# rtqichen/torchdiffeq

Measured on AMD Instinct MI355X. Metric: dopri5 RK-stages/sec at batch=65536x dim=128 (end-to-end adaptive trial steps incl. func, error norm, read-back and hos~, higher is better.
Workload: dtype f32; 1 GPU; BASELINE.json configs[1]: dopri5 adaptive, linear ODE dy/dt=Ay, batch=65536 x dim=128 fp32 per GPU, rtol=1e-7 atol=1e-9; global_batch=65536, rows_per_gpu=65536, dim=128, parallelism=batch-sharded x1, accepted=1937, rejected=2, lookahead=True, hip_graph=False

## Files before the change

include/tdeq_hip.h:

```cpp
#ifndef TDEQ_HIP_H
#define TDEQ_HIP_H

#include <stddef.h>
#include <stdint.h>

#ifdef __cplusplus
extern "C" {
#endif

#define TDEQ_ABI_VERSION 28
#define TDEQ_F32 0
#define TDEQ_F64 1
#define TDEQ_C64 2
#define TDEQ_C128 3
#define TDEQ_BF16 4
#define TDEQ_F16 5
#define TDEQ_MAX_TERMS 14
#define TDEQ_MAX_SUM_TERMS 8
#define TDEQ_MAX_DENSE_OUTPUTS 16
#define TDEQ_MAX_SEGMENTS 4096
#define TDEQ_INLINE_SEGMENTS 16
#define TDEQ_CHUNK_QUANTUM 1024

#define TDEQ_EINVAL (-1)
#define TDEQ_EWORKSPACE (-2)

typedef struct tdeq_segment {
    int64_t chunk_start;
    int64_t numel;
    double rtol;
    double atol;
} tdeq_segment;

#define TDEQ_MAX_STAGE_TIMES 16
typedef struct tdeq_step_ctrl {
    double t0;
    double dt;
    double safety;
    double ifactor;
    double dfactor;
// ... 63 lines not shown
int tdeq_stage_combine_multi_dev(const tdeq_multi_out* outs, int n_out, const void* y0, const void* acc_in,
                                 const void* const* k, int n_terms, const double* ctrl_dev, int64_t n, int dtype,
                                 void* stream);
int tdeq_stage_combine_multi_timed(const tdeq_multi_out* outs, int n_out, const void* y0, const void* acc_in,
                                   const void* const* k, int n_terms, double dt, int64_t n, int dtype, void* stream,
                                   void* start_event, void* stop_event);

int tdeq_error_norm_partial_ctrl(const void* err_partial, const void* y0, const void* y1, const void* const* k,
                                 const double* coef, int n_terms, double dt, const tdeq_segment* segs,
                                 const void* segs_dev, int n_seg, int64_t chunk, int64_t n_chunks, double* out_sumsq,
                                 double* out_nonfinite, const tdeq_step_ctrl* ctrl, double* out_ctrl, double* ctrl_dev,
                                 void* next_times, int state_in_dev, void* copy_last_k, void* workspace,
                                 size_t workspace_bytes, int dtype, void* stream);
int tdeq_stage_combine_sel(void* out, const void* y_acc, const void* f_acc, const void* y_rej, const void* f_rej,
                           double coef, const double* ctrl_dev, int64_t n, int dtype, void* stream);

int tdeq_step_controller(const double* sums, const double* nonfinite, const tdeq_segment* segs, const void* segs_dev,
                         int n_seg, double* out_sumsq, double* out_nonfinite, const tdeq_step_ctrl* ctrl,
                         double* out_ctrl, double* ctrl_dev, void* next_times, int state_in_dev, int dtype,
                         void* stream);

int tdeq_stage_combine_dev(void* out, void* err_out, const void* y0, const void* const* k, const double* coef,
                           const double* err_coef, int n_terms, const double* ctrl_dev, int64_t n, int dtype,
                           void* stream);
int tdeq_step_commit(void* y_prev, void* f_prev, void* y_cur, void* f_cur, const void* y1, const void* f1,
                     const double* ctrl_dev, int64_t n, int dtype, void* stream);

int tdeq_init_norms(int mode, const void* a, const void* b, const void* yscale,
                    const tdeq_segment* segs, const void* segs_dev, int n_seg, int64_t chunk,
                    int64_t n_chunks, double* out_sumsq, double* out_nonfinite, void* workspace, size_t workspace_bytes,
// ... 149 lines not shown
```

torchdiffeq_amd/_native.py:

```python
from __future__ import annotations

import contextlib
import ctypes
import functools
import math
import os
import threading
from typing import List, Optional, Sequence, Tuple

import numpy as np
import torch

TDEQ_ABI_VERSION = 28
TDEQ_F32, TDEQ_F64 = 0, 1
TDEQ_C64, TDEQ_C128 = 2, 3
TDEQ_BF16, TDEQ_F16 = 4, 5
TDEQ_MAX_TERMS = 14
TDEQ_INLINE_SEGMENTS = 16
TDEQ_CHUNK_QUANTUM = 1024
TDEQ_MAX_STAGE_TIMES = 16
TDEQ_MAX_DENSE_OUTPUTS = 16
TDEQ_MAX_MULTI_OUT = 4
TDEQ_MAX_GATHER = 4

_LIB_NAME = "libtdeq_hip.so"
_LIB_PATH = os.path.join(os.path.dirname(os.path.abspath(__file__)), _LIB_NAME)

_c_void_pp = ctypes.POINTER(ctypes.c_void_p)
# ... 83 lines not shown
                                                      ctypes.c_void_p, _c_void_pp, ctypes.c_int, ctypes.c_double,
                                                      ctypes.c_int64, ctypes.c_int, ctypes.c_void_p, ctypes.c_void_p,
                                                      ctypes.c_void_p]),
    "tdeq_error_norm_partial": (ctypes.c_int, [ctypes.c_void_p, ctypes.c_void_p, ctypes.c_void_p, _c_void_pp,
                                               _c_double_p, ctypes.c_int, ctypes.c_double, ctypes.POINTER(Segment),
                                               ctypes.c_void_p, ctypes.c_int, ctypes.c_int64, ctypes.c_int64,
                                               ctypes.c_void_p, ctypes.c_void_p, ctypes.c_void_p,
                                               ctypes.c_size_t, ctypes.c_int, ctypes.c_void_p]),
    "tdeq_error_norm_partial_ctrl": (ctypes.c_int, [ctypes.c_void_p, ctypes.c_void_p, ctypes.c_void_p, _c_void_pp,
                                                    _c_double_p, ctypes.c_int, ctypes.c_double,
                                                    ctypes.POINTER(Segment), ctypes.c_void_p, ctypes.c_int, ctypes.c_int64,
                                                    ctypes.c_int64, ctypes.c_void_p, ctypes.c_void_p,
                                                    ctypes.POINTER(StepCtrl), ctypes.c_void_p, ctypes.c_void_p,
                                                    ctypes.c_void_p, ctypes.c_int, ctypes.c_void_p, ctypes.c_void_p, ctypes.c_size_t,
                                                    ctypes.c_int, ctypes.c_void_p]),
    "tdeq_step_controller": (ctypes.c_int, [ctypes.c_void_p, ctypes.c_void_p, ctypes.POINTER(Segment), ctypes.c_void_p,
                                            ctypes.c_int, ctypes.c_void_p, ctypes.c_void_p,
                                            ctypes.POINTER(StepCtrl), ctypes.c_void_p, ctypes.c_void_p,
                                            ctypes.c_void_p, ctypes.c_int, ctypes.c_int, ctypes.c_void_p]),
    "tdeq_stage_combine_dev": (ctypes.c_int, [ctypes.c_void_p, ctypes.c_void_p, ctypes.c_void_p, _c_void_pp,
                                              _c_double_p, _c_double_p, ctypes.c_int, ctypes.c_void_p, ctypes.c_int64,
                                              ctypes.c_int, ctypes.c_void_p]),
    "tdeq_step_commit": (ctypes.c_int, [ctypes.c_void_p, ctypes.c_void_p, ctypes.c_void_p, ctypes.c_void_p,
                                        ctypes.c_void_p, ctypes.c_void_p, ctypes.c_void_p, ctypes.c_int64,
                                        ctypes.c_int, ctypes.c_void_p]),
    "tdeq_stage_combine_sel": (ctypes.c_int, [ctypes.c_void_p, ctypes.c_void_p, ctypes.c_void_p, ctypes.c_void_p,
                                              ctypes.c_void_p, ctypes.c_double, ctypes.c_void_p, ctypes.c_int64,
                                              ctypes.c_int, ctypes.c_void_p]),
    "tdeq_init_norms": (ctypes.c_int, [ctypes.c_int, ctypes.c_void_p, ctypes.c_void_p, ctypes.c_void_p,
                                       ctypes.POINTER(Segment), ctypes.c_void_p, ctypes.c_int,
# ... 178 lines not shown
        self.n_chunks = max(1, math.ceil(total / chunk))
        arr = (Segment * self.n_seg)()
        for i, (off, numel, rtol, atol) in enumerate(segments):
            assert off % chunk == 0, "segment offsets must be chunk aligned"
            arr[i] = Segment(off // chunk, numel, float(rtol), float(atol))
        self.segs = arr
        self.segs_dev = None
        if self.n_seg > TDEQ_INLINE_SEGMENTS:
            raw = np.frombuffer(bytes(arr), dtype=np.uint8).copy()
            self.segs_dev = torch.from_numpy(raw).to(device)
        self.workspace = torch.empty(3 * self.n_chunks, dtype=torch.float64, device=device)
        self.workspace_bytes = self.workspace.numel() * 8
        self.pinned = pinned
        self.expect = ()
        if pinned:
            self.out = torch.zeros(3 * self.n_seg + 4, dtype=torch.float64, device="cpu", pin_memory=True)
            self.out_np = self.out.numpy()
            self.out_bits = self.out_np.view(np.uint64)
        else:
            self.out = torch.zeros(3 * self.n_seg + 4, dtype=torch.float64, device=device)
            self.out_np = None
        self.out_ptr = self.out.data_ptr()
        self.bad_ptr = self.out_ptr + 16 * self.n_seg
        self.ctrl_ptr = self.out_ptr + 24 * self.n_seg
        self.ctrl_dev = torch.zeros(4, dtype=torch.float64, device=device)


class HipKernels:

    name = "hip"

    _SENTINEL = np.uint64(0x7FF8DEADBEEF0001)
    _POLL_TIMEOUT_S = 5.0

    def __init__(self, lib: ctypes.CDLL):
        self.lib = lib
        mode = os.environ.get("TDEQ_READBACK", "poll")
        if mode not in ("poll", "pinned", "copy"):
            raise ValueError(f"TDEQ_READBACK={mode!r}: expected poll | pinned | copy")
        self._mode = mode
        self._pinned = mode in ("poll", "pinned")

    def _arm(self, plan: "NormPlan", n_sum: int, ctrl: bool = False) -> None:
        if self._mode == "poll" and plan.pinned:
            n = plan.n_seg
            plan.out_bits[:n_sum * n] = self._SENTINEL
            plan.out_bits[2 * n:3 * n + (4 if ctrl else 0)] = self._SENTINEL
            plan.expect = ((0, n_sum * n), (2 * n, 3 * n + (4 if ctrl else 0)))

    _raw_stream = staticmethod(getattr(torch._C, "_cuda_getCurrentRawStream", None))
    _cur_device = staticmethod(getattr(torch._C, "_cuda_getDevice", None))

    @classmethod
    def _stream(cls) -> int:
        if cls._raw_stream is not None and cls._cur_device is not None:
            return cls._raw_stream(cls._cur_device())
        return torch.cuda.current_stream().cuda_stream

    _TLS = threading.local()
    _COEF_ARRAYS: dict = {}
    _PACK_TABLES: dict = {}

    @classmethod
# ... 212 lines not shown

    def error_norm_partial_ctrl(self, plan: NormPlan, err_partial, y0, y1, ks, coefs, dt: float, ctrl: StepCtrl,
                                next_times, state_in_dev: bool = False, copy_last_to=None) -> None:
        n = len(ks)
        ptrs = (ctypes.c_void_p * max(n, 1))(*[k.data_ptr() for k in ks])
        cf = (ctypes.c_double * max(n, 1))(*coefs)
        self._arm(plan, 1, ctrl=True)
        _check(self.lib.tdeq_error_norm_partial_ctrl(
            err_partial.data_ptr(), y0.data_ptr(), y1.data_ptr(), ptrs, cf, n, dt, plan.segs,
            plan.segs_dev.data_ptr() if plan.segs_dev is not None else None, plan.n_seg, plan.chunk,
            plan.n_chunks, plan.out_ptr, plan.bad_ptr, ctypes.byref(ctrl), plan.ctrl_ptr, plan.ctrl_dev.data_ptr(),
            next_times.data_ptr(), 1 if state_in_dev else 0, None if copy_last_to is None else copy_last_to.data_ptr(),
            plan.workspace.data_ptr(), plan.workspace_bytes, dtype_code(y0.dtype), self._stream()),
            "tdeq_error_norm_partial_ctrl")

    def step_controller(self, plan: NormPlan, sums_plan: NormPlan, numel_plan: NormPlan, ctrl: StepCtrl, next_times,
                        dtype: torch.dtype, state_in_dev: bool = False) -> None:
        assert not sums_plan.pinned and sums_plan.n_seg == plan.n_seg == numel_plan.n_seg
        self._arm(plan, 1, ctrl=True)
        _check(self.lib.tdeq_step_controller(
            sums_plan.out_ptr, sums_plan.bad_ptr, numel_plan.segs,
            numel_plan.segs_dev.data_ptr() if numel_plan.segs_dev is not None else None, plan.n_seg, plan.out_ptr,
            plan.bad_ptr, ctypes.byref(ctrl), plan.ctrl_ptr, plan.ctrl_dev.data_ptr(), next_times.data_ptr(),
            1 if state_in_dev else 0, dtype_code(dtype), self._stream()), "tdeq_step_controller")

    def read_ctrl(self, plan: NormPlan) -> Tuple[bool, float, float, List[float]]:
        n = plan.n_seg
        v = self._read_out(plan)
        return v[3 * n] != 0.0, v[3 * n + 1], v[3 * n + 2], v[2 * n:3 * n]

    def stage_combine_dev(self, out, err_out, y0, ks, coefs, err_coefs, plan: NormPlan) -> None:
        ptrs, cf, n = self._terms(ks, coefs)
        ef = None if err_coefs is None else (ctypes.c_double * n)(*err_coefs)
        _check(self.lib.tdeq_stage_combine_dev(out.data_ptr(), None if err_out is None else err_out.data_ptr(),
                                               y0.data_ptr(), ptrs, cf, ef, n, plan.ctrl_dev.data_ptr(), y0.numel(),
                                               dtype_code(y0.dtype), self._stream()), "tdeq_stage_combine_dev")

    def step_commit(self, y_prev, f_prev, y_cur, f_cur, y1, f1, plan: NormPlan) -> None:
        _check(self.lib.tdeq_step_commit(y_prev.data_ptr(), f_prev.data_ptr(), y_cur.data_ptr(), f_cur.data_ptr(),
                                         y1.data_ptr(), f1.data_ptr(), plan.ctrl_dev.data_ptr(), y_cur.numel(),
                                         dtype_code(y_cur.dtype), self._stream()), "tdeq_step_commit")

    def arm_readback(self, plan: NormPlan, n_sum: int = 1, ctrl: bool = True) -> None:
# ... 442 lines not shown
```

torchdiffeq_amd/csrc/tdeq_abi.hip:

```cpp
#include <hip/hip_runtime.h>
#include <hip/hip_ext.h>

#include <cstdlib>

#include "tdeq_kernels.hpp"
#include "tdeq_kernels_complex.hpp"
#include "tdeq_kernels_lp.hpp"

namespace {
using namespace tdeq;

constexpr int64_t kMaxGrid = 1 << 16;

inline unsigned stream_grid(int64_t n_items, int items_per_block) {
    int64_t g = (n_items + items_per_block - 1) / items_per_block;
    const int64_t cap = kMaxGrid;
    if (g > cap) g = cap;
    if (g < 1) g = 1;
    return (unsigned)g;
}

inline bool aligned16(const void* p) { return (reinterpret_cast<uintptr_t>(p) & 15u) == 0; }

inline int check_launch() {
// ... 530 lines not shown
    const bool vec = aligned16(out) && aligned16(y_acc) && aligned16(f_acc) && aligned16(y_rej) && aligned16(f_rej);
    if (vec) {
        const dim3 g(stream_grid(n / L, kBlock)), b(kBlock);
        switch (stream_policy((int64_t)3 * n * (int64_t)sizeof(T))) {
            case 1: hipLaunchKernelGGL((stage_combine_sel_kernel<T, true, 1>), g, b, 0, s, a); break;
            case 2: hipLaunchKernelGGL((stage_combine_sel_kernel<T, true, 2>), g, b, 0, s, a); break;
            case 3: hipLaunchKernelGGL((stage_combine_sel_kernel<T, true, 3>), g, b, 0, s, a); break;
            default: hipLaunchKernelGGL((stage_combine_sel_kernel<T, true, 0>), g, b, 0, s, a);
        }
    } else {
        hipLaunchKernelGGL((stage_combine_sel_kernel<T, false>), dim3(stream_grid(n, kBlock)), dim3(kBlock), 0, s, a);
    }
    return check_launch();
}

template <typename T>
int launch_init(int mode, const void* a_, const void* b_, const void* y_, const SegTable& st,
                double* out_sumsq, double* out_bad, double* ws, hipStream_t s) {
    InitArgs<T> a;
    a.a = static_cast<const T*>(a_);
    a.b = static_cast<const T*>(b_);
    a.y = static_cast<const T*>(y_);
    a.st = st;
    a.part0 = ws;
    a.part1 = ws + st.n_chunks;
    a.part_bad = ws + 2 * st.n_chunks;
    const bool vec = aligned16(a_) && aligned16(b_) && aligned16(y_);
    const dim3 g((unsigned)st.n_chunks), b(kBlock);
    if (mode == 0) {
        if (vec) hipLaunchKernelGGL((init_norms_kernel<T, 0, true>), g, b, 0, s, a);
// ... 706 lines not shown
    const int e = fill_segtable(st, segs, segs_dev, n_seg, chunk, n_chunks);
    if (e) return e;
    if (workspace_bytes < tdeq_workspace_bytes(n_chunks)) return TDEQ_EWORKSPACE;
    hipStream_t s = static_cast<hipStream_t>(stream);
    double* ws = static_cast<double*>(workspace);
    const CtrlBundle cb{ctrl, out_ctrl, ctrl_dev, next_times, state_in_dev ? 1 : 0};
    if (dtype == TDEQ_C64)
        return dispatch_cplx_error_partial<float>(err_partial, y0, y1, k, coef, n_terms, dt, st, out_sumsq, out_nonfinite, ws, &cb, s);
    if (dtype == TDEQ_C128)
        return dispatch_cplx_error_partial<double>(err_partial, y0, y1, k, coef, n_terms, dt, st, out_sumsq, out_nonfinite, ws, &cb, s);
    return dtype == TDEQ_F32
               ? dispatch_error_partial<float>(err_partial, y0, y1, k, coef, n_terms, dt, st, out_sumsq, out_nonfinite, ws, &cb, s, copy_last_k)
               : dispatch_error_partial<double>(err_partial, y0, y1, k, coef, n_terms, dt, st, out_sumsq, out_nonfinite, ws, &cb, s, copy_last_k);
}

int tdeq_step_controller(const double* sums, const double* nonfinite, const tdeq_segment* segs, const void* segs_dev,
                         int n_seg, double* out_sumsq, double* out_nonfinite, const tdeq_step_ctrl* ctrl,
                         double* out_ctrl, double* ctrl_dev, void* next_times, int state_in_dev, int dtype,
                         void* stream) {
    if (!sums || !nonfinite || !segs || !out_sumsq || !out_nonfinite || !ctrl || !out_ctrl || !ctrl_dev ||
        !next_times || bad_dtype(dtype))
        return TDEQ_EINVAL;
    if (ctrl->n_times < 1 || ctrl->n_times > TDEQ_MAX_STAGE_TIMES || ctrl->n_norm_seg < 0 || ctrl->n_norm_seg > n_seg)
        return TDEQ_EINVAL;
    SegTable st;
    const int e = fill_segtable(st, segs, segs_dev, n_seg, TDEQ_CHUNK_QUANTUM, 1);
    if (e) return e;
    CtrlArgs a;
    a.part_sumsq = nullptr;
    a.part_bad = nullptr;
// ... 394 lines not shown
```

torchdiffeq_amd/csrc/tdeq_kernels.hpp:

```cpp
#pragma once

#include <hip/hip_runtime.h>
#include <stdint.h>

#include "tdeq_hip.h"

namespace tdeq {

constexpr int kBlock = 256;
constexpr int kWave = 64;

typedef float f32x4 __attribute__((ext_vector_type(4)));
typedef double f64x2 __attribute__((ext_vector_type(2)));

template <typename T> struct VecOf;
template <> struct VecOf<float> { using type = f32x4; static constexpr int L = 4; };
template <> struct VecOf<double> { using type = f64x2; static constexpr int L = 2; };

template <typename V> __device__ __forceinline__ V vabs(V v);
template <> __device__ __forceinline__ f32x4 vabs(f32x4 v) {
    return f32x4{__builtin_fabsf(v.x), __builtin_fabsf(v.y), __builtin_fabsf(v.z), __builtin_fabsf(v.w)};
}
template <> __device__ __forceinline__ f64x2 vabs(f64x2 v) {
    return f64x2{__builtin_fabs(v.x), __builtin_fabs(v.y)};
// ... 800 lines not shown
    float tt;
    if ((c.alpha_is_one >> i) & 1u) tt = ctl_prev16(t1T, tkind);
    else tt = ctl_rnd16(t0T + ctl_rnd16((float)c.alpha[i] * dtT, tkind), tkind);
    return ctl_bits16((float)c.time_sign * tt, tkind);
}

template <typename T>
__device__ __forceinline__ T ctl_stage_time(const tdeq_step_ctrl& c, double t0n, double dtn, int i) {
    const T t0T = (T)t0n, dtT = (T)dtn, t1T = (T)(t0n + dtn);
    T tt;
    if ((c.alpha_is_one >> i) & 1u) tt = ctl_prev(t1T);
    else tt = t0T + (T)c.alpha[i] * dtT;
    return (T)c.time_sign * tt;
}

constexpr int kCtrlInlineSegments = 4;
template <int NS>
__global__ __launch_bounds__(kBlock) void norm_finalize_ctrl_kernel(const CtrlArgs a) {
    __shared__ double red[2 * NS * (kBlock / kWave)];
    __shared__ double seg_val[2][NS];
    __shared__ double next_step[2];
    const int n_seg = a.st.n_seg;
    if (a.presummed) {
        const double* sums = a.in_sumsq ? a.in_sumsq : a.out_sumsq;
        if (a.in_sumsq)
            for (int s = threadIdx.x; s < n_seg; s += kBlock) {
                a.out_sumsq[s] = a.in_sumsq[s];
                a.out_bad[s] = a.in_bad[s];
            }
        double part[2] = {0.0, 0.0};
// ... 69 lines not shown
    if (threadIdx.x == 0) {
        const double dev_t0 = a.ctrl_dev[2], dev_dt = a.ctrl_dev[3];
        const double arg_t0 = c.t0, arg_dt = c.dt;
        const double step_t0 = a.state_in_dev ? dev_t0 : arg_t0;
        const double step_dt = a.state_in_dev ? dev_dt : arg_dt;
        double val = 0.0;
        if (a.presummed) val = seg_val[0][0];
        for (int s = 0; s < c.n_norm_seg && s < n_seg && !a.presummed; ++s) {
            const int64_t numel = a.st.inl[s].numel;
            if (numel == 0) continue;
            const double v = (s == 0 && numel == 1 && c.leading_abs && a.ratio_kind >= 2)
                                 ? (double)ctl_rnd16((float)seg_val[0][s], a.ratio_kind)
                                 : ctl_seg_norm(seg_val[0][s], numel, a.ratio_kind);
            val = ctl_nan_max(val, v);
        }
        const double ratio = a.ratio_kind == 1 ? (double)(float)val : val;
        bool accept = ratio <= 1.0;
        if (step_dt > c.max_step) accept = false;
        if (step_dt <= c.min_step) accept = true;
        double dt_next;
        if (ratio == 0.0) {
            dt_next = step_dt * c.ifactor;
        } else {
            const double dfactor = ratio < 1.0 ? 1.0 : c.dfactor;
            const double scaled = c.safety / pow(ratio, c.exponent);
            dt_next = step_dt * ctl_nan_min(c.ifactor, ctl_nan_max(scaled, dfactor));
        }
        dt_next = ctl_clamp(dt_next, c.min_step, c.max_step);
        const double t0n = accept ? step_t0 + step_dt : step_t0;
        double dtn = dt_next;
        if (!__builtin_isfinite(dtn)) dtn = c.min_step;
        dtn = ctl_clamp(dtn, c.min_step, c.max_step);
        a.ctrl_dev[0] = accept ? 1.0 : 0.0;
        a.ctrl_dev[1] = ctl_round_T(dtn, a.is_f32) * c.time_sign;
        a.ctrl_dev[2] = t0n;
        a.ctrl_dev[3] = dtn;
        next_step[0] = t0n;
        next_step[1] = dtn;
        a.out_ctrl[0] = accept ? 1.0 : 0.0;
        a.out_ctrl[1] = dt_next;
        a.out_ctrl[2] = ratio;
        a.out_ctrl[3] = t0n;
    }
    __syncthreads();
    const int i = threadIdx.x;
    if (i < c.n_times) {
        if (a.is_f32 >= 2) static_cast<uint16_t*>(a.next_times)[i] = ctl_stage_time16(c, next_step[0], next_step[1], i, a.is_f32);
// ... 187 lines not shown
    const E* __restrict__ y = reinterpret_cast<const E*>(ys);
    const E* __restrict__ f = reinterpret_cast<const E*>(fs);
    if (i0 < ne) {
        if (!accept) {
            y_spec = ld_stream<POLICY>(y + i0);
            f_spec = ld_stream<POLICY>(f + i0);
        }
        st_stream<POLICY>(out + i0, y_spec + f_spec * c);
    }
    for (int64_t i = i0 + stride; i < ne; i += stride)
        st_stream<POLICY>(out + i, ld_stream<POLICY>(y + i) + ld_stream<POLICY>(f + i) * c);
    if (VEC) {
        const int64_t t = ne * L + threadIdx.x;
        if (blockIdx.x == 0 && t < a.n) a.out[t] = ys[t] + fs[t] * c;
    }
}

template <typename T, int NT>
struct DenseArgs {
    T* out;
    const T* y0;
    const T* y1;
    const T* f0;
    const T* f1;
    const T* k[NT];
    T c[NT];
    T dt;
    T x;
    int64_t n;
};
// ... 616 lines not shown
```

torchdiffeq_amd/solvers/adaptive.py:

```python
from __future__ import annotations

import bisect
import collections
import math
import os
import warnings
from typing import List, Optional, Sequence

import numpy as np
import torch

from .. import _native
from .._graph import (_AUTO_CAPTURE_AFTER_STEPS, _AUTO_MIN_GRID_STEPS, _GRAPH_AUTO_MAX_ELEMENTS,
                     _GRAPH_MODE_MAX_ELEMENTS, _CaptureFailed, _DtCell, _GraphStep, _capture, _graph_request,
                     _held_tensor_ptrs, _reusable_across_solves, _scalar_state, _side_effect_fingerprint, _side_stream,
                     _request_is_explicit, _stream_is_capturing, clear_graph_cache)
from .._scalars import is_low, power, rdiv, scalar_type
from ..autodiff import Ops, stitch
from ..misc import (BuiltinNorm, OdeFunc, Perturb, StateLayout, component_norm, find_event, handle_unused_kwargs, rms_norm,
                   vector_tolerances)
from ..misc import _null_callback as _null
from ..tableaus import (ADAPTIVE_HEUN, ADAPTIVE_TABLEAUS, BOSH3, CARRY_DEFAULT_ON, DOPRI5, DOPRI8, FEHLBERG2, FUSE_ODEINT, TSIT5, SparseRow,
                       Tableau, adams_coefficients, carry_plan, fused_lead, row_by_row_plan)
from ._common import _nan_max, _nan_min, _clamp, _norm_value, _as_float, optimal_step_size, optimal_step_size_in, _StepShadow, _NoShadow, _NO_SHADOW
# ... 199 lines not shown
            and func.time_dtype == y0.dtype and dist_sync is None
        device_ctrl = (getattr(self.kernels, "device_controller", True)
                       and (self._fuse is not None or self._whole_row_ctrl or self._vec_ctrl)
                       and (isinstance(self.norm, BuiltinNorm) or self._vec_ctrl)
                       and len(self._beta) <= _native.TDEQ_MAX_STAGE_TIMES and n_norm_seg >= 0
                       and self.step_t is None and self.jump_t is None and (self._sync is None or sync_dev)
                       and self._wide)
        self._plan_dev = self._plan_glob = None
        if device_ctrl and self._sync is not None:
            segs = self.layout.segments(rtol, atol)
            self._plan_dev = _native.NormPlan(segs, self.layout.total, self.layout.chunk, y0.device, pinned=False)
            self._plan_glob = self.kernels.make_plan([(off, gn, rt, at) for (off, _, rt, at), gn in
                                                      zip(segs, self._numels)], self.layout.total,
                                                     self.layout.chunk, y0.device)
        self._lookahead = device_ctrl and os.environ.get("TDEQ_LOOKAHEAD", "1") != "0"
        wanted, auto = _graph_request(hip_graph)
        self._graph_auto = auto
        self._graph_explicit = _request_is_explicit(hip_graph)
        if wanted and _stream_is_capturing():
            wanted = False
        self._graph_watch = wanted and auto and y0.device.type == "cuda"
        self._auto = None
        self._auto_steps = 0
        self._hold_pre = False
        self.hip_graph = wanted and device_ctrl and self._sync is None and y0.device.type == "cuda" \
            and (not self._vec_ctrl or getattr(self.kernels, "vec_ctrl_in_graph", False)) \
            and hasattr(self.kernels, "stage_combine_dev") \
            and self.layout.total <= (_GRAPH_AUTO_MAX_ELEMENTS if auto else _GRAPH_MODE_MAX_ELEMENTS) * \
            (2 if (y0.element_size() == 2 and not auto) else 1)
        if wanted and not auto and not self.hip_graph and hip_graph is not None:
# ... 467 lines not shown
        err_partial = held.pop(R, None)
        assert not held
        err = self._c_err
        return yi, k, err_partial, ((plan.err_idx, plan.err_coef) if err_partial is not None else (err.idx, err.coef))

    def _error_ratio(self, y0, f0, y1, k, err_partial, err_rem, t0, dt, t1, dt_signed, lookahead):
        func, kern = self.func, self.kernels
        builtin_norm, vec_fused = self._partial_norm()
        ks, coefs = [k[j] for j in err_rem[0]], err_rem[1]
        vec_ctrl = self._vec_ctrl and not builtin_norm and (err_partial is None or vec_fused)
        if lookahead and ((err_partial is not None and (builtin_norm or vec_ctrl))
                          or (self._whole_row_ctrl and builtin_norm) or vec_ctrl):
            ctrl = self._ctrl
            ctrl.t0, ctrl.dt = t0, dt
            tnext = torch.empty(ctrl.n_times, dtype=func.time_dtype, device=y0.device)
            if vec_ctrl:
                kern.error_norm_vec_ctrl(self.plan, y0, y1, ks, coefs, dt_signed, self._vec_fused[0], self._vec_fused[1],
                                         ctrl, tnext, **({} if err_partial is None else {"partial": err_partial}))
            elif err_partial is None:
                kern.error_norm_ctrl(self.plan, y0, y1, ks, coefs, dt_signed, ctrl, tnext)
            elif self._sync is None:
                kern.error_norm_partial_ctrl(self.plan, err_partial, y0, y1, ks, coefs, dt_signed, ctrl, tnext)
            else:
                kern.error_norm_partial(self._plan_dev, err_partial, y0, y1, ks, coefs, dt_signed)
                self._sync.reduce_device(self._plan_dev.out, self.plan.n_seg)
                kern.step_controller(self.plan, self._plan_dev, self._plan_glob, ctrl, tnext, y0.dtype)
            if t1 < self._t_end and not self._hold_pre and not self._last_trial:
                yi_n = torch.empty_like(y0)
                kern.stage_combine_sel(yi_n, y1, k[-1], y0, f0, self._beta[0].coef[0], self.plan)
                tn = tnext.unbind(0)
                self._pre = (yi_n, tn, func.eval_at(tn[0], yi_n))
            accept_dev, dt_next_dev, error_ratio, bad = kern.read_ctrl(self.plan)
            return error_ratio, any(b != 0 for b in bad), (accept_dev, dt_next_dev)
        if not builtin_norm:
            return self._user_norm_ratio(y0, y1, k, dt_signed, err_partial, err_rem) + (None,)
        if err_partial is not None:
            kern.error_norm_partial(self.plan, err_partial, y0, y1, ks, coefs, dt_signed)
        else:
            kern.error_norm(self.plan, y0, y1, ks, coefs, dt_signed)
        sumsq, _, bad = self._read_norms()
        return self._segment_norm(sumsq, bad), any(b != 0 for b in bad), None

    def _commit(self, accept_step, dt_next, y0, y1, k, t0, dt, t1, dt_signed, dsh, dsh_signed, on_step_t, on_jump_t,
                y1_nonfinite) -> None:
        func = self.func
        if accept_step:
            if func.callback_accept_step is not _null:
# ... 118 lines not shown
```

Measured before the change: 18320 RK-stages/s.

## Fuse error norm, step controller and next-stage select into one grid kernel

Adds a single kernel launched with one workgroup per CU that computes the partial error norm and runs the step-controller decision. The other workgroups spin on an agent-scope handoff flag until that decision is published, then write the lookahead stage input by selecting between the accepted and rejected state. Chunks of y1 and k still held in registers are reused, which removes a separate select launch and part of its reread of y1 and k. A spin limit with a gave-up flag falls back to the separate launches, and a size window plus an environment variable decide when the fused path is used. The risk is that the spin-wait handoff stalls or deadlocks if workgroups are not all co-resident.

```diff
diff --git a/include/tdeq_hip.h b/include/tdeq_hip.h
--- a/include/tdeq_hip.h
+++ b/include/tdeq_hip.h
@@ -8,7 +8,7 @@
 extern "C" {
 #endif
 
-#define TDEQ_ABI_VERSION 28
+#define TDEQ_ABI_VERSION 29
 #define TDEQ_F32 0
 #define TDEQ_F64 1
 #define TDEQ_C64 2
@@ -24,6 +24,7 @@
 
 #define TDEQ_EINVAL (-1)
 #define TDEQ_EWORKSPACE (-2)
+#define TDEQ_ENOTAPPLICABLE (-3)
 
 typedef struct tdeq_segment {
     int64_t chunk_start;
@@ -117,6 +118,16 @@
                                  size_t workspace_bytes, int dtype, void* stream);
 int tdeq_stage_combine_sel(void* out, const void* y_acc, const void* f_acc, const void* y_rej, const void* f_rej,
                            double coef, const double* ctrl_dev, int64_t n, int dtype, void* stream);
+
+int tdeq_error_norm_partial_ctrl_sel(const void* err_partial, const void* y0, const void* y1, const void* const* k,
+                                     const double* coef, int n_terms, double dt, const tdeq_segment* segs,
+                                     const void* segs_dev, int n_seg, int64_t chunk, int64_t n_chunks,
+                                     double* out_sumsq, double* out_nonfinite, const tdeq_step_ctrl* ctrl,
+                                     double* out_ctrl, double* ctrl_dev, void* next_times, int state_in_dev,
+                                     void* copy_last_k, void* workspace, size_t workspace_bytes, int dtype, void* stream,
+                                     void* out, const void* y_acc, const void* f_acc, const void* y_rej,
+                                     const void* f_rej, double sel_coef, int64_t n, void* handoff, uint32_t epoch,
+                                     int max_workgroups, uint32_t max_spins);
 
 int tdeq_step_controller(const double* sums, const double* nonfinite, const tdeq_segment* segs, const void* segs_dev,
                          int n_seg, double* out_sumsq, double* out_nonfinite, const tdeq_step_ctrl* ctrl,
diff --git a/torchdiffeq_amd/_native.py b/torchdiffeq_amd/_native.py
--- a/torchdiffeq_amd/_native.py
+++ b/torchdiffeq_amd/_native.py
@@ -6,12 +6,14 @@
 import math
 import os
 import threading
+import warnings
 from typing import List, Optional, Sequence, Tuple
 
 import numpy as np
 import torch
 
-TDEQ_ABI_VERSION = 28
+TDEQ_ABI_VERSION = 29
+TDEQ_ENOTAPPLICABLE = -3
 TDEQ_F32, TDEQ_F64 = 0, 1
 TDEQ_C64, TDEQ_C128 = 2, 3
 TDEQ_BF16, TDEQ_F16 = 4, 5
@@ -125,6 +127,16 @@
                                                     ctypes.POINTER(StepCtrl), ctypes.c_void_p, ctypes.c_void_p,
                                                     ctypes.c_void_p, ctypes.c_int, ctypes.c_void_p, ctypes.c_void_p, ctypes.c_size_t,
                                                     ctypes.c_int, ctypes.c_void_p]),
+    "tdeq_error_norm_partial_ctrl_sel": (ctypes.c_int, [ctypes.c_void_p, ctypes.c_void_p, ctypes.c_void_p, _c_void_pp,
+                                                        _c_double_p, ctypes.c_int, ctypes.c_double,
+                                                        ctypes.POINTER(Segment), ctypes.c_void_p, ctypes.c_int,
+                                                        ctypes.c_int64, ctypes.c_int64, ctypes.c_void_p, ctypes.c_void_p,
+                                                        ctypes.POINTER(StepCtrl), ctypes.c_void_p, ctypes.c_void_p,
+                                                        ctypes.c_void_p, ctypes.c_int, ctypes.c_void_p, ctypes.c_void_p,
+                                                        ctypes.c_size_t, ctypes.c_int, ctypes.c_void_p,
+                                                        ctypes.c_void_p, ctypes.c_void_p, ctypes.c_void_p, ctypes.c_void_p,
+                                                        ctypes.c_void_p, ctypes.c_double, ctypes.c_int64, ctypes.c_void_p,
+                                                        ctypes.c_uint32, ctypes.c_int, ctypes.c_uint32]),
     "tdeq_step_controller": (ctypes.c_int, [ctypes.c_void_p, ctypes.c_void_p, ctypes.POINTER(Segment), ctypes.c_void_p,
                                             ctypes.c_int, ctypes.c_void_p, ctypes.c_void_p,
                                             ctypes.POINTER(StepCtrl), ctypes.c_void_p, ctypes.c_void_p,
@@ -333,16 +345,19 @@
         self.pinned = pinned
         self.expect = ()
         if pinned:
-            self.out = torch.zeros(3 * self.n_seg + 4, dtype=torch.float64, device="cpu", pin_memory=True)
+            self.out = torch.zeros(3 * self.n_seg + 5, dtype=torch.float64, device="cpu", pin_memory=True)
             self.out_np = self.out.numpy()
             self.out_bits = self.out_np.view(np.uint64)
         else:
-            self.out = torch.zeros(3 * self.n_seg + 4, dtype=torch.float64, device=device)
+            self.out = torch.zeros(3 * self.n_seg + 5, dtype=torch.float64, device=device)
             self.out_np = None
         self.out_ptr = self.out.data_ptr()
         self.bad_ptr = self.out_ptr + 16 * self.n_seg
         self.ctrl_ptr = self.out_ptr + 24 * self.n_seg
         self.ctrl_dev = torch.zeros(4, dtype=torch.float64, device=device)
+        self.handoff: dict = {}
+        self.fused_pending = False
+        self.gave_up = False
 
 
 class HipKernels:
@@ -360,12 +375,14 @@
         self._mode = mode
         self._pinned = mode in ("poll", "pinned")
 
-    def _arm(self, plan: "NormPlan", n_sum: int, ctrl: bool = False) -> None:
+    def _arm(self, plan: "NormPlan", n_sum: int, ctrl: bool = False, fused: bool = False) -> None:
+        plan.fused_pending = fused
         if self._mode == "poll" and plan.pinned:
             n = plan.n_seg
+            n_ctrl = (5 if fused else 4) if ctrl else 0
             plan.out_bits[:n_sum * n] = self._SENTINEL
-            plan.out_bits[2 * n:3 * n + (4 if ctrl else 0)] = self._SENTINEL
-            plan.expect = ((0, n_sum * n), (2 * n, 3 * n + (4 if ctrl else 0)))
+            plan.out_bits[2 * n:3 * n + n_ctrl] = self._SENTINEL
+            plan.expect = ((0, n_sum * n), (2 * n, 3 * n + n_ctrl))
 
     _raw_stream = staticmethod(getattr(torch._C, "_cuda_getCurrentRawStream", None))
     _cur_device = staticmethod(getattr(torch._C, "_cuda_getDevice", None))
@@ -608,6 +625,54 @@
             plan.workspace.data_ptr(), plan.workspace_bytes, dtype_code(y0.dtype), self._stream()),
             "tdeq_error_norm_partial_ctrl")
 
+    FUSED_TAIL_FROM = 1 << 22
+    FUSED_TAIL_BELOW = 3 << 22
+    fused_tail_max_spins = 0
+    _fused_tail_warned = False
+
+    @classmethod
+    def fused_tail_wanted(cls, numel: int) -> bool:
+        env = os.environ.get("TDEQ_FUSED_TAIL")
+        if env is not None and env != "":
+            return env != "0"
+        return cls.FUSED_TAIL_FROM <= numel < cls.FUSED_TAIL_BELOW
+
+    @classmethod
+    def warn_fused_tail_gave_up(cls) -> None:
+        if not cls._fused_tail_warned:
+            cls._fused_tail_warned = True
+            warnings.warn("torchdiffeq_amd: a workgroup of the fused step tail ran out of polls while waiting for the step "
+                          "controller (the GPU is shared with other work?); the step was redone with the separate launches, "
+                          "which this solve uses from here on", RuntimeWarning, stacklevel=3)
+
+    def error_norm_partial_ctrl_sel(self, plan: NormPlan, err_partial, y0, y1, ks, coefs, dt: float, ctrl: StepCtrl,
+                                    next_times, out, y_rej, f_rej, sel_coef: float, max_workgroups: int = 0,
+                                    max_spins: Optional[int] = None) -> bool:
+        n = len(ks)
+        if n < 1:
+            return False
+        ptrs = (ctypes.c_void_p * n)(*[k.data_ptr() for k in ks])
+        cf = (ctypes.c_double * n)(*coefs)
+        hand = plan.handoff.get(max_workgroups)
+        if hand is None or hand[1] == 0xFFFFFFFF:
+            hand = plan.handoff[max_workgroups] = [torch.zeros(160, dtype=torch.int32, device=y0.device), 0]
+        epoch = hand[1] + 1
+        self._arm(plan, 1, ctrl=True, fused=True)
+        code = self.lib.tdeq_error_norm_partial_ctrl_sel(
+            err_partial.data_ptr(), y0.data_ptr(), y1.data_ptr(), ptrs, cf, n, dt, plan.segs,
+            plan.segs_dev.data_ptr() if plan.segs_dev is not None else None, plan.n_seg, plan.chunk, plan.n_chunks,
+            plan.out_ptr, plan.bad_ptr, ctypes.byref(ctrl), plan.ctrl_ptr, plan.ctrl_dev.data_ptr(), next_times.data_ptr(),
+            0, None, plan.workspace.data_ptr(), plan.workspace_bytes, dtype_code(y0.dtype), self._stream(),
+            out.data_ptr(), y1.data_ptr(), ks[-1].data_ptr(), y_rej.data_ptr(), f_rej.data_ptr(), sel_coef, out.numel(),
+            hand[0].data_ptr(), epoch, max_workgroups, self.fused_tail_max_spins if max_spins is None else max_spins)
+        if code == TDEQ_ENOTAPPLICABLE:
+            plan.fused_pending = False
+            plan.expect = ()
+            return False
+        _check(code, "tdeq_error_norm_partial_ctrl_sel")
+        hand[1] = epoch
+        return True
+
     def step_controller(self, plan: NormPlan, sums_plan: NormPlan, numel_plan: NormPlan, ctrl: StepCtrl, next_times,
                         dtype: torch.dtype, state_in_dev: bool = False) -> None:
         assert not sums_plan.pinned and sums_plan.n_seg == plan.n_seg == numel_plan.n_seg
@@ -621,6 +686,8 @@
     def read_ctrl(self, plan: NormPlan) -> Tuple[bool, float, float, List[float]]:
         n = plan.n_seg
         v = self._read_out(plan)
+        plan.gave_up = bool(plan.fused_pending and v[3 * n + 4] != 0.0)
+        plan.fused_pending = False
         return v[3 * n] != 0.0, v[3 * n + 1], v[3 * n + 2], v[2 * n:3 * n]
 
     def stage_combine_dev(self, out, err_out, y0, ks, coefs, err_coefs, plan: NormPlan) -> None:
diff --git a/torchdiffeq_amd/csrc/tdeq_abi.hip b/torchdiffeq_amd/csrc/tdeq_abi.hip
--- a/torchdiffeq_amd/csrc/tdeq_abi.hip
+++ b/torchdiffeq_amd/csrc/tdeq_abi.hip
@@ -568,6 +568,73 @@
     return check_launch();
 }
 
+inline int device_cu_count() {
+    static int cus[64] = {0};
+    int dev = 0;
+    if (hipGetDevice(&dev) != hipSuccess || dev < 0 || dev >= 64) return 0;
+    if (cus[dev] == 0) {
+        int v = 0;
+        if (hipDeviceGetAttribute(&v, hipDeviceAttributeMultiprocessorCount, dev) != hipSuccess) return 0;
+        cus[dev] = v;
+    }
+    return cus[dev];
+}
+
+struct TailSel {
+    void* out;
+    const void* y_rej;
+    const void* f_rej;
+    double coef;
+    void* handoff;
+    uint32_t epoch;
+    int max_workgroups;
+    uint32_t max_spins;
+};
+
+template <typename T, int NT>
+int launch_norm_ctrl_sel(const void* partial, const void* y0, const void* y1, const void* const* k, const double* coef,
+                         double dt, const tdeq_segment& seg, int64_t chunk, int64_t n_chunks, double* out_sumsq,
+                         double* out_bad, double* ws, const CtrlBundle& cb, const TailSel& t, hipStream_t s) {
+    constexpr int L = VecOf<T>::L;
+    const int vpc = (int)(chunk / (L * kBlock));
+    if (chunk != (int64_t)vpc * L * kBlock || (vpc != 4 / L && vpc != 8 / L)) return TDEQ_ENOTAPPLICABLE;
+    NormCtrlSelArgs<T, NT> a;
+    a.partial = static_cast<const T*>(partial);
+    a.y0 = static_cast<const T*>(y0);
+    a.y1 = static_cast<const T*>(y1);
+    const T dtT = (T)dt;
+    for (int j = 0; j < NT; ++j) {
+        a.k[j] = static_cast<const T*>(k[j]);
+        a.c[j] = (T)coef[j] * dtT;
+    }
+    a.numel = seg.numel;
+    a.n_chunks = n_chunks;
+    a.rtol = seg.rtol;
+    a.atol = seg.atol;
+    a.part_sumsq = ws;
+    a.part_bad = ws + 2 * n_chunks;
+    a.ctl = *cb.ctrl;
+    a.out_sumsq = out_sumsq;
+    a.out_bad = out_bad;
+    a.out_ctrl = cb.out_ctrl;
+    a.ctrl_dev = cb.ctrl_dev;
+    a.next_times = cb.next_times;
+    a.out = static_cast<T*>(t.out);
+    a.y_rej = static_cast<const T*>(t.y_rej);
+    a.f_rej = static_cast<const T*>(t.f_rej);
+    a.coef = (T)t.coef;
+    a.hand = static_cast<unsigned*>(t.handoff);
+    a.epoch = t.epoch;
+    a.max_spins = t.max_spins;
+    int g = device_cu_count();
+    if (g < 1) return TDEQ_ENOTAPPLICABLE;
+    if (t.max_workgroups > 0 && t.max_workgroups < g) g = t.max_workgroups;
+    const dim3 grid((unsigned)g), block(kTailBlock);
+    if (vpc == 4 / L) hipLaunchKernelGGL((norm_ctrl_sel_kernel<T, NT, 4 / L>), grid, block, 0, s, a);
+    else hipLaunchKernelGGL((norm_ctrl_sel_kernel<T, NT, 8 / L>), grid, block, 0, s, a);
+    return check_launch();
+}
+
 template <typename T>
 int launch_init(int mode, const void* a_, const void* b_, const void* y_, const SegTable& st,
                 double* out_sumsq, double* out_bad, double* ws, hipStream_t s) {
@@ -1304,6 +1371,48 @@
                : dispatch_error_partial<double>(err_partial, y0, y1, k, coef, n_terms, dt, st, out_sumsq, out_nonfinite, ws, &cb, s, copy_last_k);
 }
 
+int tdeq_error_norm_partial_ctrl_sel(const void* err_partial, const void* y0, const void* y1, const void* const* k,
+                                     const double* coef, int n_terms, double dt, const tdeq_segment* segs,
+                                     const void* segs_dev, int n_seg, int64_t chunk, int64_t n_chunks,
+                                     double* out_sumsq, double* out_nonfinite, const tdeq_step_ctrl* ctrl,
+                                     double* out_ctrl, double* ctrl_dev, void* next_times, int state_in_dev,
+                                     void* copy_last_k, void* workspace, size_t workspace_bytes, int dtype, void* stream,
+                                     void* out, const void* y_acc, const void* f_acc, const void* y_rej,
+                                     const void* f_rej, double sel_coef, int64_t n, void* handoff, uint32_t epoch,
+                                     int max_workgroups, uint32_t max_spins) {
+    if (!err_partial || !y0 || !y1 || !out_sumsq || !out_nonfinite || !workspace) return TDEQ_EINVAL;
+    if (!ctrl || !out_ctrl || !ctrl_dev || !next_times || !handoff || epoch == 0) return TDEQ_EINVAL;
+    if (!out || !y_acc || !f_acc || !y_rej || !f_rej || n < 0) return TDEQ_EINVAL;
+    if (n_terms < 0 || n_terms > 2 || (n_terms > 0 && (!k || !coef))) return TDEQ_EINVAL;
+    for (int j = 0; j < n_terms; ++j) if (!k[j]) return TDEQ_EINVAL;
+    if (ctrl->n_times < 1 || ctrl->n_times > TDEQ_MAX_STAGE_TIMES || ctrl->n_norm_seg < 0 || ctrl->n_norm_seg > n_seg)
+        return TDEQ_EINVAL;
+    if (dtype != TDEQ_F32 && dtype != TDEQ_F64) return (bad_dtype(dtype) && !lp_dtype(dtype)) ? TDEQ_EINVAL : TDEQ_ENOTAPPLICABLE;
+    SegTable st;
+    const int e = fill_segtable(st, segs, segs_dev, n_seg, chunk, n_chunks);
+    if (e) return e;
+    if (workspace_bytes < tdeq_workspace_bytes(n_chunks)) return TDEQ_EWORKSPACE;
+    if (state_in_dev || copy_last_k || n_seg != 1 || st.inl[0].chunk_start != 0 || n_terms < 1 || n < 1) return TDEQ_ENOTAPPLICABLE;
+    if (st.inl[0].numel != n || n_chunks != (n + chunk - 1) / chunk || y_acc != y1 || f_acc != k[n_terms - 1]) return TDEQ_ENOTAPPLICABLE;
+    bool vec = aligned16(err_partial) && aligned16(y0) && aligned16(y1) && aligned16(out) && aligned16(y_rej) && aligned16(f_rej);
+    for (int j = 0; j < n_terms; ++j) vec = vec && aligned16(k[j]);
+    if (!vec) return TDEQ_ENOTAPPLICABLE;
+    const int64_t esz = dtype == TDEQ_F32 ? 4 : 8;
+    if (stream_policy((int64_t)(n_terms + 3) * n_chunks * chunk * esz) != 0 || stream_policy((int64_t)3 * n * esz) != 0)
+        return TDEQ_ENOTAPPLICABLE;
+    hipStream_t s = static_cast<hipStream_t>(stream);
+    double* ws = static_cast<double*>(workspace);
+    const CtrlBundle cb{ctrl, out_ctrl, ctrl_dev, next_times, 0};
+    const TailSel t{out, y_rej, f_rej, sel_coef, handoff, epoch, max_workgroups, max_spins};
+    if (dtype == TDEQ_F32)
+        return n_terms == 1
+                   ? launch_norm_ctrl_sel<float, 1>(err_partial, y0, y1, k, coef, dt, st.inl[0], chunk, n_chunks, out_sumsq, out_nonfinite, ws, cb, t, s)
+                   : launch_norm_ctrl_sel<float, 2>(err_partial, y0, y1, k, coef, dt, st.inl[0], chunk, n_chunks, out_sumsq, out_nonfinite, ws, cb, t, s);
+    return n_terms == 1
+               ? launch_norm_ctrl_sel<double, 1>(err_partial, y0, y1, k, coef, dt, st.inl[0], chunk, n_chunks, out_sumsq, out_nonfinite, ws, cb, t, s)
+               : launch_norm_ctrl_sel<double, 2>(err_partial, y0, y1, k, coef, dt, st.inl[0], chunk, n_chunks, out_sumsq, out_nonfinite, ws, cb, t, s);
+}
+
 int tdeq_step_controller(const double* sums, const double* nonfinite, const tdeq_segment* segs, const void* segs_dev,
                          int n_seg, double* out_sumsq, double* out_nonfinite, const tdeq_step_ctrl* ctrl,
                          double* out_ctrl, double* ctrl_dev, void* next_times, int state_in_dev, int dtype,
diff --git a/torchdiffeq_amd/csrc/tdeq_kernels.hpp b/torchdiffeq_amd/csrc/tdeq_kernels.hpp
--- a/torchdiffeq_amd/csrc/tdeq_kernels.hpp
+++ b/torchdiffeq_amd/csrc/tdeq_kernels.hpp
@@ -838,6 +838,39 @@
     return (T)c.time_sign * tt;
 }
 
+struct CtrlDecision {
+    bool accept;
+    double dt_next;
+    double ratio;
+    double t0n, dtn;
+};
+__device__ __forceinline__ CtrlDecision ctl_decide(const tdeq_step_ctrl& c, double val, int ratio_kind, double step_t0,
+                                                   double step_dt) {
+    CtrlDecision d;
+    const double ratio = ratio_kind == 1 ? (double)(float)val : val;
+    bool accept = ratio <= 1.0;
+    if (step_dt > c.max_step) accept = false;
+    if (step_dt <= c.min_step) accept = true;
+    double dt_next;
+    if (ratio == 0.0) {
+        dt_next = step_dt * c.ifactor;
+    } else {
+        const double dfactor = ratio < 1.0 ? 1.0 : c.dfactor;
+        const double scaled = c.safety / pow(ratio, c.exponent);
+        dt_next = step_dt * ctl_nan_min(c.ifactor, ctl_nan_max(scaled, dfactor));
+    }
+    dt_next = ctl_clamp(dt_next, c.min_step, c.max_step);
+    double dtn = dt_next;
+    if (!__builtin_isfinite(dtn)) dtn = c.min_step;
+    dtn = ctl_clamp(dtn, c.min_step, c.max_step);
+    d.accept = accept;
+    d.dt_next = dt_next;
+    d.ratio = ratio;
+    d.t0n = accept ? step_t0 + step_dt : step_t0;
+    d.dtn = dtn;
+    return d;
+}
+
 constexpr int kCtrlInlineSegments = 4;
 template <int NS>
 __global__ __launch_bounds__(kBlock) void norm_finalize_ctrl_kernel(const CtrlArgs a) {
@@ -937,23 +970,9 @@
                                  : ctl_seg_norm(seg_val[0][s], numel, a.ratio_kind);
             val = ctl_nan_max(val, v);
         }
-        const double ratio = a.ratio_kind == 1 ? (double)(float)val : val;
-        bool accept = ratio <= 1.0;
-        if (step_dt > c.max_step) accept = false;
-        if (step_dt <= c.min_step) accept = true;
-        double dt_next;
-        if (ratio == 0.0) {
-            dt_next = step_dt * c.ifactor;
-        } else {
-            const double dfactor = ratio < 1.0 ? 1.0 : c.dfactor;
-            const double scaled = c.safety / pow(ratio, c.exponent);
-            dt_next = step_dt * ctl_nan_min(c.ifactor, ctl_nan_max(scaled, dfactor));
-        }
-        dt_next = ctl_clamp(dt_next, c.min_step, c.max_step);
-        const double t0n = accept ? step_t0 + step_dt : step_t0;
-        double dtn = dt_next;
-        if (!__builtin_isfinite(dtn)) dtn = c.min_step;
-        dtn = ctl_clamp(dtn, c.min_step, c.max_step);
+        const CtrlDecision d = ctl_decide(c, val, a.ratio_kind, step_t0, step_dt);
+        const bool accept = d.accept;
+        const double dt_next = d.dt_next, ratio = d.ratio, t0n = d.t0n, dtn = d.dtn;
         a.ctrl_dev[0] = accept ? 1.0 : 0.0;
         a.ctrl_dev[1] = ctl_round_T(dtn, a.is_f32) * c.time_sign;
         a.ctrl_dev[2] = t0n;
@@ -1171,6 +1190,313 @@
         const int64_t t = ne * L + threadIdx.x;
         if (blockIdx.x == 0 && t < a.n) a.out[t] = ys[t] + fs[t] * c;
     }
+}
+
+constexpr int kTailBlock = 1024;
+constexpr int kTailTeams = kTailBlock / kBlock;
+template <typename T, int NT>
+struct TailShape {
+    static constexpr int keep = (sizeof(T) == 4 && NT == 1) ? 8 : 4;
+    static constexpr int batch = keep == 8 ? 1 : 2;
+};
+constexpr int kTailSlots = 16;
+constexpr unsigned kTailMaxSpins = 1u << 16;
+enum { kHandTicket = 0, kHandFlag = 32, kHandGaveUp = 64, kHandDone = 96, kHandPub = 128, kHandWords = 160 };
+
+template <typename T, int NT>
+struct NormCtrlSelArgs {
+    const T* partial;
+    const T* y0;
+    const T* y1;
+    const T* k[NT];
+    T c[NT];
+    int64_t numel, n_chunks;
+    double rtol, atol;
+    double* part_sumsq;
+    double* part_bad;
+    tdeq_step_ctrl ctl;
+    double* out_sumsq;
+    double* out_bad;
+    double* out_ctrl;
+    double* ctrl_dev;
+    void* next_times;
+    T* out;
+    const T* y_rej;
+    const T* f_rej;
+    T coef;
+    unsigned* hand;
+    unsigned epoch;
+    unsigned max_spins;
+};
+
+__device__ __forceinline__ void tail_drain() { __builtin_amdgcn_s_waitcnt(0x0F70); }
+__device__ __forceinline__ void tail_pub_store(double* p, double v) {
+    __hip_atomic_store(p, v, __ATOMIC_RELAXED, __HIP_MEMORY_SCOPE_AGENT);
+}
+__device__ __forceinline__ double tail_pub_load(const double* p) {
+    return __hip_atomic_load(p, __ATOMIC_RELAXED, __HIP_MEMORY_SCOPE_AGENT);
+}
+
+template <typename T, int NT, int VPC>
+__global__ __launch_bounds__(kTailBlock) void norm_ctrl_sel_kernel(const NormCtrlSelArgs<T, NT> a) {
+    using V = typename VecOf<T>::type;
+    constexpr int L = VecOf<T>::L;
+    constexpr int W = kBlock / kWave;
+    constexpr int KC = TailShape<T, NT>::keep / VPC;
+    constexpr int JB = VPC < TailShape<T, NT>::batch ? VPC : TailShape<T, NT>::batch;
+    static_assert(TailShape<T, NT>::keep % VPC == 0 && VPC % JB == 0, "kept vectors are whole chunk rounds");
+    __shared__ double red[kTailSlots][kTailTeams][2][W];
+    __shared__ double fin[2 * W];
+    __shared__ double bc[4];
+    __shared__ int state[2];
+    const int tid = threadIdx.x, team = tid / kBlock, lt = tid % kBlock, lane = tid & (kWave - 1), wv = lt / kWave;
+    const int64_t G = gridDim.x;
+    const int64_t per = (a.n_chunks + G - 1) / G;
+    const int64_t c_lo = (int64_t)blockIdx.x * per < a.n_chunks ? (int64_t)blockIdx.x * per : a.n_chunks;
+    const int64_t c_hi = c_lo + per < a.n_chunks ? c_lo + per : a.n_chunks;
+    const int64_t rounds = (per + kTailTeams - 1) / kTailTeams;
+    constexpr int64_t cv = (int64_t)VPC * kBlock;
+    constexpr int64_t chunk = cv * L;
+    const T rtol = (T)a.rtol, atol = (T)a.atol;
+    const V* __restrict__ pe = reinterpret_cast<const V*>(a.partial);
+    const V* __restrict__ y0 = reinterpret_cast<const V*>(a.y0);
+    const V* __restrict__ y1 = reinterpret_cast<const V*>(a.y1);
+
+    V yk[KC][VPC], fk[KC][VPC];
+    int64_t r = 0;
+    auto valid_of = [&](int64_t b) -> int64_t {
+        const int64_t v = a.numel - b * chunk;
+        return (b >= c_hi || v < 0) ? 0 : (v > chunk ? chunk : v);
+    };
+    auto chunk_step = [&](V (&yc)[VPC], V (&fc)[VPC]) {
+        const int64_t b = c_lo + r * kTailTeams + team;
+        const int64_t valid = valid_of(b), nv = valid / L;
+        double acc0 = 0.0, acc1 = 0.0;
+        if (nv == cv) {
+#pragma unroll
+            for (int j0 = 0; j0 < VPC; j0 += JB) {
+                V v1[JB], kv[JB][NT], e[JB], v0[JB];
+#pragma unroll
+                for (int u = 0; u < JB; ++u) {
+                    const int64_t gi = b * cv + lt + (j0 + u) * kBlock;
+                    v1[u] = y1[gi];
+#pragma unroll
+                    for (int q = 0; q < NT; ++q) kv[u][q] = reinterpret_cast<const V*>(a.k[q])[gi];
+                    e[u] = pe[gi];
+                    v0[u] = y0[gi];
+                }
+#pragma unroll
+                for (int u = 0; u < JB; ++u) {
+#pragma unroll
+                    for (int q = 0; q < NT; ++q) e[u] = e[u] + kv[u][q] * a.c[q];
+#pragma unroll
+                    for (int q = 0; q < L; ++q) tol_accumulate<T>(e[u][q], v0[u][q], v1[u][q], rtol, atol, acc0, acc1);
+                    yc[j0 + u] = v1[u];
+                    fc[j0 + u] = kv[u][NT - 1];
+                }
+            }
+        } else {
+#pragma unroll
+            for (int jj = 0; jj < VPC; ++jj) {
+                const int64_t i = lt + jj * kBlock;
+                if (i < nv) {
+                    const int64_t gi = b * cv + i;
+                    const V v1 = y1[gi];
+                    V kv[NT];
+#pragma unroll
+                    for (int q = 0; q < NT; ++q) kv[q] = reinterpret_cast<const V*>(a.k[q])[gi];
+                    V e = pe[gi];
+                    const V v0 = y0[gi];
+#pragma unroll
+                    for (int q = 0; q < NT; ++q) e = e + kv[q] * a.c[q];
+#pragma unroll
+                    for (int q = 0; q < L; ++q) tol_accumulate<T>(e[q], v0[q], v1[q], rtol, atol, acc0, acc1);
+                    yc[jj] = v1;
+                    fc[jj] = kv[NT - 1];
+                }
+            }
+            const int64_t base = b * chunk;
+            for (int64_t t = nv * L + lt; t < valid; t += kBlock) {
+                T e = a.partial[base + t];
+#pragma unroll
+                for (int q = 0; q < NT; ++q) e = e + a.k[q][base + t] * a.c[q];
+                tol_accumulate<T>(e, a.y0[base + t], a.y1[base + t], rtol, atol, acc0, acc1);
+            }
+        }
+        acc0 = wave_sum(acc0);
+        acc1 = wave_sum(acc1);
+        const int slot = (int)(r % kTailSlots);
+        if (lane == 0) {
+            red[slot][team][0][wv] = acc0;
+            red[slot][team][1][wv] = acc1;
+        }
+        if (slot == kTailSlots - 1 || r == rounds - 1) {
+            __syncthreads();
+            if (tid < (slot + 1) * kTailTeams) {
+                const int sl = tid / kTailTeams, tm = tid % kTailTeams;
+                const int64_t bb = c_lo + (r - slot + sl) * kTailTeams + tm;
+                if (bb < c_hi) {
+                    double s0 = red[sl][tm][0][0], s1 = red[sl][tm][1][0];
+#pragma unroll
+                    for (int w = 1; w < W; ++w) {
+                        s0 += red[sl][tm][0][w];
+                        s1 += red[sl][tm][1][w];
+                    }
+                    tail_pub_store(a.part_sumsq + bb, s0);
+                    tail_pub_store(a.part_bad + bb, s1);
+                }
+            }
+            __syncthreads();
+        }
+        ++r;
+    };
+#pragma unroll
+    for (int s = 0; s < KC; ++s)
+        if (s < rounds) chunk_step(yk[s], fk[s]);
+    for (int64_t s = KC; s < rounds; ++s) {
+        V yd[VPC], fd[VPC];
+        chunk_step(yd, fd);
+    }
+
+    if (tid < kWave) tail_drain();
+    if (tid == 0) {
+        const unsigned old = __hip_atomic_fetch_add(a.hand + kHandTicket, 1u, __ATOMIC_RELAXED, __HIP_MEMORY_SCOPE_AGENT);
+        state[0] = (old + 1u == a.epoch * (unsigned)G);
+        state[1] = 1;
+    }
+    __syncthreads();
+    const tdeq_step_ctrl& c = a.ctl;
+    constexpr int tkind = sizeof(T) == 4 ? 1 : 0;
+    if (state[0]) {
+        double a0 = 0.0, a1 = 0.0;
+        if (tid < kBlock) {
+            int64_t i = tid;
+            for (; i + (kFinBatch - 1) * kBlock < a.n_chunks; i += kFinBatch * kBlock) {
+                double v[kFinBatch], w[kFinBatch];
+#pragma unroll
+                for (int u = 0; u < kFinBatch; ++u) {
+                    v[u] = tail_pub_load(a.part_sumsq + i + u * kBlock);
+                    w[u] = tail_pub_load(a.part_bad + i + u * kBlock);
+                }
+#pragma unroll
+                for (int u = 0; u < kFinBatch; ++u) {
+                    a0 += v[u];
+                    a1 += w[u];
+                }
+            }
+            for (; i < a.n_chunks; i += kBlock) {
+                a0 += tail_pub_load(a.part_sumsq + i);
+                a1 += tail_pub_load(a.part_bad + i);
+            }
+        }
+        a0 = wave_sum(a0);
+        a1 = wave_sum(a1);
+        if (tid < kBlock && lane == 0) {
+            fin[wv] = a0;
+            fin[W + wv] = a1;
+        }
+        __syncthreads();
+        if (tid == 0) {
+            double s0 = fin[0], s1 = fin[W];
+#pragma unroll
+            for (int w = 1; w < W; ++w) {
+                s0 += fin[w];
+                s1 += fin[W + w];
+            }
+            double val = 0.0;
+            if (c.n_norm_seg > 0 && a.numel != 0) val = ctl_nan_max(val, ctl_seg_norm(s0, a.numel, tkind));
+            const CtrlDecision d = ctl_decide(c, val, tkind, c.t0, c.dt);
+            const double acc_w = d.accept ? 1.0 : 0.0, dt_w = ctl_round_T(d.dtn, tkind) * c.time_sign;
+            double* pub = reinterpret_cast<double*>(a.hand + kHandPub);
+            tail_pub_store(a.ctrl_dev + 0, acc_w);
+            tail_pub_store(a.ctrl_dev + 1, dt_w);
+            tail_pub_store(a.ctrl_dev + 2, d.t0n);
+            tail_pub_store(a.ctrl_dev + 3, d.dtn);
+            tail_pub_store(pub + 0, acc_w);
+            tail_pub_store(pub + 1, d.dt_next);
+            tail_pub_store(pub + 2, d.ratio);
+            tail_pub_store(pub + 3, d.t0n);
+            tail_pub_store(pub + 4, s0);
+            tail_pub_store(pub + 5, s1);
+            tail_drain();
+            __hip_atomic_store(a.hand + kHandFlag, a.epoch, __ATOMIC_RELAXED, __HIP_MEMORY_SCOPE_AGENT);
+            bc[0] = d.t0n;
+            bc[1] = d.dtn;
+            bc[2] = acc_w;
+            bc[3] = dt_w;
+        }
+        __syncthreads();
+        if (tid < c.n_times) {
+            if (tkind) static_cast<float*>(a.next_times)[tid] = ctl_stage_time<float>(c, bc[0], bc[1], tid);
+            else static_cast<double*>(a.next_times)[tid] = ctl_stage_time<double>(c, bc[0], bc[1], tid);
+        }
+    } else {
+        if (tid == 0) {
+            const unsigned spins = a.max_spins ? a.max_spins : kTailMaxSpins;
+            bool seen = false;
+            for (unsigned p = 0; p < spins; ++p) {
+                if (__hip_atomic_load(a.hand + kHandFlag, __ATOMIC_RELAXED, __HIP_MEMORY_SCOPE_AGENT) == a.epoch) {
+                    seen = true;
+                    break;
+                }
+                __builtin_amdgcn_s_sleep(2);
+            }
+            __builtin_amdgcn_fence(__ATOMIC_ACQUIRE, "wavefront");
+            if (seen) {
+                bc[2] = tail_pub_load(a.ctrl_dev + 0);
+                bc[3] = tail_pub_load(a.ctrl_dev + 1);
+            } else {
+                __hip_atomic_fetch_or(a.hand + kHandGaveUp, 1u, __ATOMIC_RELAXED, __HIP_MEMORY_SCOPE_AGENT);
+                state[1] = 0;
+            }
+        }
+        __syncthreads();
+    }
+    if (tid == 0) {
+        tail_drain();
+        const unsigned old = __hip_atomic_fetch_add(a.hand + kHandDone, 1u, __ATOMIC_RELAXED, __HIP_MEMORY_SCOPE_AGENT);
+        if (old + 1u == a.epoch * (unsigned)G) {
+            const double* pub = reinterpret_cast<const double*>(a.hand + kHandPub);
+            const double p0 = tail_pub_load(pub + 0), p1 = tail_pub_load(pub + 1), p2 = tail_pub_load(pub + 2);
+            const double p3 = tail_pub_load(pub + 3), p4 = tail_pub_load(pub + 4), p5 = tail_pub_load(pub + 5);
+            const unsigned gave = __hip_atomic_load(a.hand + kHandGaveUp, __ATOMIC_RELAXED, __HIP_MEMORY_SCOPE_AGENT);
+            a.out_sumsq[0] = p4;
+            a.out_bad[0] = p5;
+            a.out_ctrl[0] = p0;
+            a.out_ctrl[1] = p1;
+            a.out_ctrl[2] = p2;
+            a.out_ctrl[3] = p3;
+            a.out_ctrl[4] = gave ? 1.0 : 0.0;
+        }
+    }
+    if (!state[1]) return;
+
+    const bool accept = bc[2] != 0.0;
+    const T cs = a.coef * (T)bc[3];
+    const T* ys = accept ? a.y1 : a.y_rej;
+    const T* fs = accept ? a.k[NT - 1] : a.f_rej;
+    const V* __restrict__ yv = reinterpret_cast<const V*>(ys);
+    const V* __restrict__ fv = reinterpret_cast<const V*>(fs);
+    V* __restrict__ out = reinterpret_cast<V*>(a.out);
+    auto out_chunk = [&](int64_t rr, const V (&yc)[VPC], const V (&fc)[VPC], bool kept) {
+        const int64_t b = c_lo + rr * kTailTeams + team;
+        const int64_t nv = valid_of(b) / L;
+#pragma unroll
+        for (int jj = 0; jj < VPC; ++jj) {
+            const int64_t i = lt + jj * kBlock;
+            if (i < nv) {
+                const int64_t gi = b * cv + i;
+                if (kept) out[gi] = yc[jj] + fc[jj] * cs;
+                else out[gi] = yv[gi] + fv[gi] * cs;
+            }
+        }
+    };
+#pragma unroll
+    for (int s = 0; s < KC; ++s)
+        if (s < rounds) out_chunk(s, yk[s], fk[s], accept);
+    for (int64_t s = KC; s < rounds; ++s) out_chunk(s, yk[0], fk[0], false);
+    const int64_t t = (a.numel / L) * L + tid;
+    if (blockIdx.x == 0 && t < a.numel) a.out[t] = ys[t] + fs[t] * cs;
 }
 
 template <typename T, int NT>
diff --git a/torchdiffeq_amd/solvers/adaptive.py b/torchdiffeq_amd/solvers/adaptive.py
--- a/torchdiffeq_amd/solvers/adaptive.py
+++ b/torchdiffeq_amd/solvers/adaptive.py
@@ -237,6 +237,7 @@
                                                       zip(segs, self._numels)], self.layout.total,
                                                      self.layout.chunk, y0.device)
         self._lookahead = device_ctrl and os.environ.get("TDEQ_LOOKAHEAD", "1") != "0"
+        self._fused_tail = True
         wanted, auto = _graph_request(hip_graph)
         self._graph_auto = auto
         self._graph_explicit = _request_is_explicit(hip_graph)
@@ -734,23 +735,41 @@
             ctrl = self._ctrl
             ctrl.t0, ctrl.dt = t0, dt
             tnext = torch.empty(ctrl.n_times, dtype=func.time_dtype, device=y0.device)
+            another = t1 < self._t_end and not self._hold_pre and not self._last_trial
+            fused = False
             if vec_ctrl:
                 kern.error_norm_vec_ctrl(self.plan, y0, y1, ks, coefs, dt_signed, self._vec_fused[0], self._vec_fused[1],
                                          ctrl, tnext, **({} if err_partial is None else {"partial": err_partial}))
             elif err_partial is None:
                 kern.error_norm_ctrl(self.plan, y0, y1, ks, coefs, dt_signed, ctrl, tnext)
             elif self._sync is None:
-                kern.error_norm_partial_ctrl(self.plan, err_partial, y0, y1, ks, coefs, dt_signed, ctrl, tnext)
+                if (self._fused_tail and another and ks and hasattr(kern, "error_norm_partial_ctrl_sel")
+                        and kern.fused_tail_wanted(y0.numel())):
+                    yi_n = torch.empty_like(y0)
+                    fused = kern.error_norm_partial_ctrl_sel(self.plan, err_partial, y0, y1, ks, coefs, dt_signed, ctrl, tnext,
+                                                             yi_n, y0, f0, self._beta[0].coef[0])
+                if not fused:
+                    kern.error_norm_partial_ctrl(self.plan, err_partial, y0, y1, ks, coefs, dt_signed, ctrl, tnext)
             else:
                 kern.error_norm_partial(self._plan_dev, err_partial, y0, y1, ks, coefs, dt_signed)
                 self._sync.reduce_device(self._plan_dev.out, self.plan.n_seg)
                 kern.step_controller(self.plan, self._plan_dev, self._plan_glob, ctrl, tnext, y0.dtype)
-            if t1 < self._t_end and not self._hold_pre and not self._last_trial:
+            if another:
+                if not fused:
+                    yi_n = torch.empty_like(y0)
+                    kern.stage_combine_sel(yi_n, y1, k[-1], y0, f0, self._beta[0].coef[0], self.plan)
+                tn = tnext.unbind(0)
+                self._pre = (yi_n, tn, func.eval_at(tn[0], yi_n))
+            accept_dev, dt_next_dev, error_ratio, bad = kern.read_ctrl(self.plan)
+            if fused and self.plan.gave_up:
+                kern.warn_fused_tail_gave_up()
+                self._fused_tail = False
+                kern.error_norm_partial_ctrl(self.plan, err_partial, y0, y1, ks, coefs, dt_signed, ctrl, tnext)
                 yi_n = torch.empty_like(y0)
                 kern.stage_combine_sel(yi_n, y1, k[-1], y0, f0, self._beta[0].coef[0], self.plan)
                 tn = tnext.unbind(0)
                 self._pre = (yi_n, tn, func.eval_at(tn[0], yi_n))
-            accept_dev, dt_next_dev, error_ratio, bad = kern.read_ctrl(self.plan)
+                accept_dev, dt_next_dev, error_ratio, bad = kern.read_ctrl(self.plan)
             return error_ratio, any(b != 0 for b in bad), (accept_dev, dt_next_dev)
         if not builtin_norm:
             return self._user_norm_ratio(y0, y1, k, dt_signed, err_partial, err_rem) + (None,)
```

Measured after the change: 17560 RK-stages/s. 4.1% lower.
